# zhiqwang/yolort

Measured on NVIDIA H100. Metric: images/sec end-to-end (letterbox->NMS), higher is better.
Workload: dtype f16

## Files before the change

yolort_b200/csrc/conv_sm90.cu:

```cuda
#include <cstdlib>

#include "common.cuh"
#include "conv_sm90.h"
#include "conv_epilogue.cuh"
#include "conv_chain.cuh"
#include "decode_common.cuh"

namespace yb {

namespace {

constexpr int kMaxStages = 12;
__host__ __device__ constexpr int tile_rows(int groups) { return 64 * groups; }
__host__ __device__ constexpr int cta_threads(int groups) { return 128 * (1 + groups); }
__host__ __device__ constexpr int stage_buf_bytes(int groups) { return tile_rows(groups) * 128; }
constexpr int kStageBufs = 2;
constexpr int kMaxBlockN = 256;
constexpr size_t kSmemBudget = 216 * 1024;
constexpr size_t kStaticSmem = (2 * kMaxStages + 2) * 8 + 2 * kMaxBlockN * 4;
constexpr uint32_t kConsumerBar = 1;

struct ConvKernelParams {
  int M, block_n, block_k;
  int ksize, chunks, num_k_iters;
  int mode;
  int HoWo, Wo, stride, pad;
  int stages;
  int kpg;
  int b_resident;
  uint32_t b_res_bytes;
  int n_tiles, num_tiles;
  int full_tiles, split, num_tasks;
  int ctas;
  int groups;
  int store_cols;
  int bias_len;
  int kk_last;
  uint32_t a_stage_bytes, b_stage_bytes;
  const float* bias;
  EpilogueParams ep;
  ChainParams ch;
  int decode_on;
  int dec_H, dec_W;
  yb_head_decode dec;
};

template <int kGroups>
__device__ __forceinline__ void consumer_sync() { named_bar_sync(kConsumerBar, 128 * kGroups); }

struct ConvTask {
  int m_tile, n_tile, piece, split;
};
template <bool kSplits>
__device__ __forceinline__ ConvTask conv_task(const ConvKernelParams& p, int t) {
  ConvTask k;
  int tile = t;
  k.piece = 0;
  k.split = 1;
  if (kSplits && t >= p.full_tiles) {
    const int u = t - p.full_tiles;
    const int q = u / p.n_tiles;
    tile = p.full_tiles + (q / p.split) * p.n_tiles + (u - q * p.n_tiles);
    k.piece = q % p.split;
    k.split = p.split;
  }
  k.m_tile = tile / p.n_tiles;
  k.n_tile = tile - k.m_tile * p.n_tiles;
  return k;
}

template <bool kBf16, int kW>
__device__ __forceinline__ int stage_mmas(float* acc, const ConvKernelParams& p, uint32_t a_lo0, uint32_t a_step16,
                                          uint32_t b_lo0, uint32_t b_step16, uint64_t ab_hi, int cnt, int ch, int kk,
                                          bool first) {
  for (int j = 0; j < cnt; ++j) {
    const int kc = ch == p.chunks - 1 ? p.kk_last : kk;
    for (int k = 0; k < kc; ++k)
      wgmma_mma<kBf16, kW>(acc, desc_lohi(a_lo0 + j * a_step16 + 2 * k, ab_hi), desc_lohi(b_lo0 + j * b_step16 + 2 * k, ab_hi),
                           !first || (j | k) != 0);
    if (++ch == p.chunks) ch = 0;
  }
  return ch;
}

template <int kN>
__device__ __forceinline__ void decode_fragment(const yb_head_decode& D, const float* acc, const float* s_bias,
                                                const FragRows& fr, int dec_H, int dec_W, float* head, uint32_t wg_bar,
                                                int lane) {
  constexpr int kMaxA = 4;
  const int K = D.n_classes + 5;
  const int q2 = 2 * (lane & 3);
#pragma unroll
  for (int j = 0; j < kN / 8; ++j) {
    {
#pragma unroll
      for (int i = 0; i < 4; ++i) {
        const int col = 8 * j + q2 + (i & 1);
        const int a = col / K, r = col - a * K;
        if (a < D.n_anchors && r < 5) head[fr.loc[i >> 1] * 20 + a * 5 + r] = acc[4 * j + i] + s_bias[col];
      }
    }
  }
  named_bar_sync(wg_bar, 128);
  float obj[2][kMaxA];
  bool pass[2][kMaxA];
  uint32_t emitted[2] = {0u, 0u};
#pragma unroll
  for (int rr = 0; rr < 2; ++rr) {
#pragma unroll
    for (int a = 0; a < kMaxA; ++a) {
      obj[rr][a] = a < D.n_anchors ? sigmoidf_ref(head[fr.loc[rr] * 20 + a * 5 + 4]) : 0.f;
      pass[rr][a] = a < D.n_anchors && fr.ok[rr] && obj[rr][a] > D.score_thresh;
    }
  }
  int n_img[2], py[2], px[2];
  const int hw = dec_H * dec_W;
#pragma unroll
  for (int rr = 0; rr < 2; ++rr) {
    n_img[rr] = static_cast<int>(fr.row[rr] / hw);
    const int rem = static_cast<int>(fr.row[rr] - static_cast<long long>(n_img[rr]) * hw);
    py[rr] = rem / dec_W;
    px[rr] = rem - py[rr] * dec_W;
  }
  const bool any_pass = pass[0][0] || pass[0][1] || pass[0][2] || pass[0][3] || pass[1][0] || pass[1][1] ||
                        pass[1][2] || pass[1][3];
  if (any_pass) {
#pragma unroll
    for (int j = 0; j < kN / 8; ++j) {
      {
#pragma unroll
        for (int i = 0; i < 4; ++i) {
          const int rr = i >> 1;
          const int col = 8 * j + q2 + (i & 1);
          const int a = col / K, r = col - a * K;
          const bool pa = a == 0 ? pass[rr][0] : (a == 1 ? pass[rr][1] : (a == 2 ? pass[rr][2] : (a == 3 && pass[rr][3])));
          if (pa && r >= 5) {
            const float oa = a == 0 ? obj[rr][0] : (a == 1 ? obj[rr][1] : (a == 2 ? obj[rr][2] : obj[rr][3]));
            const float score = __fmul_rn(sigmoidf_ref(acc[4 * j + i] + s_bias[col]), oa);
            if (score > D.score_thresh) {
              const int anchor_flat = D.level_start + (a * dec_H + py[rr]) * dec_W + px[rr];
              emit_candidate(D.keys, D.img_count, D.cap_per_image, n_img[rr], anchor_flat, D.n_classes, r - 5, score);
              emitted[rr] |= 1u << a;
            }
          }
        }
      }
    }
  }
#pragma unroll
  for (int rr = 0; rr < 2; ++rr) {
    emitted[rr] |= __shfl_xor_sync(0xffffffffu, emitted[rr], 1);
    emitted[rr] |= __shfl_xor_sync(0xffffffffu, emitted[rr], 2);
    if ((lane & 3) == 0 && emitted[rr]) {
      const float* h = head + fr.loc[rr] * 20;
      for (int a = 0; a < D.n_anchors; ++a) {
        if (!((emitted[rr] >> a) & 1u)) continue;
        const int anchor_flat = D.level_start + (a * dec_H + py[rr]) * dec_W + px[rr];
        const float4 b = decode_box(sigmoidf_ref(h[a * 5 + 0]), sigmoidf_ref(h[a * 5 + 1]), sigmoidf_ref(h[a * 5 + 2]),
                                    sigmoidf_ref(h[a * 5 + 3]), px[rr], py[rr], D.stride_px, D.anchors_px[2 * a],
                                    D.anchors_px[2 * a + 1]);
        reinterpret_cast<float4*>(D.boxes)[static_cast<long long>(n_img[rr]) * D.anchors_per_image + anchor_flat] = b;
        atomicMax(&D.img_maxc[n_img[rr]], float_to_ordered_int(fmaxf(fmaxf(b.x, b.y), fmaxf(b.z, b.w))));
      }
    }
  }
  named_bar_sync(wg_bar, 128);
}

template <bool kBf16, int kN, bool kDecode, int kN2, int kCtas, int kGroups = 2>
__global__ void __launch_bounds__(cta_threads(kGroups), kCtas)
conv_wgmma_kernel(const __grid_constant__ CUtensorMap tmap_a, const __grid_constant__ CUtensorMap tmap_b,
                  const __grid_constant__ CUtensorMap tmap_out, const __grid_constant__ CUtensorMap tmap_w2,
                  const __grid_constant__ CUtensorMap tmap_out2, const __grid_constant__ CUtensorMap tmap_a64,
                  const __grid_constant__ CUtensorMap tmap_out64, const ConvKernelParams p) {
  static_assert(kGroups == 2 || (kGroups == 1 && kCtas == 2 && !kDecode), "one consumer warpgroup: two CTAs, no decode");
  constexpr bool kChain = kN2 != 0;
  constexpr int kAcc = (kN > kN2 ? kN : kN2) / 2;
  constexpr int kBlockM = tile_rows(kGroups);
  constexpr int kStageBufBytes = stage_buf_bytes(kGroups);
  constexpr bool kSplits = !kDecode && !kChain && kN == 128;
  constexpr bool kRowHalves = kSplits && kGroups == 2;
  extern __shared__ uint8_t smem_raw[];
  __shared__ __align__(8) uint64_t full_bar[kMaxStages];
  __shared__ __align__(8) uint64_t empty_bar[kMaxStages];
  __shared__ __align__(8) uint64_t b_full;
  __shared__ __align__(8) uint64_t w2_full;
  __shared__ __align__(16) float s_bias[kMaxBlockN];
  __shared__ __align__(16) float s_bias2[kChain ? kMaxBlockN : 4];

  uint8_t* tiles = reinterpret_cast<uint8_t*>(
      (reinterpret_cast<uintptr_t>(smem_raw) + 1023) & ~static_cast<uintptr_t>(1023));
  const uint32_t stage_bytes = p.kpg * (p.a_stage_bytes + (p.b_resident ? 0u : p.b_stage_bytes));
  uint8_t* b_res = tiles + static_cast<size_t>(p.stages) * stage_bytes;
  uint8_t* staging = b_res + p.b_res_bytes;
  uint8_t* w2_res = staging + kStageBufs * kStageBufBytes;

  const int warp = threadIdx.x >> 5;
  const int lane = threadIdx.x & 31;

  if (threadIdx.x == 0) {
    tma_prefetch_desc(&tmap_a);
    tma_prefetch_desc(&tmap_b);
    tma_prefetch_desc(&tmap_out);
    for (int s = 0; s < p.stages; ++s) {
      mbar_init(&full_bar[s], 1);
      mbar_init(&empty_bar[s], kGroups);
    }
    mbar_init(&b_full, 1);
    mbar_init(&w2_full, 1);
    mbar_fence_init();
  }
  __syncthreads();

  if (threadIdx.x == 0 && p.b_resident) {
    const uint32_t b_bytes = p.block_n * p.block_k * 2;
    const int n0 = (blockIdx.x % p.n_tiles) * p.block_n;
    mbar_expect_tx(&b_full, p.num_k_iters * b_bytes);
    for (int it = 0; it < p.num_k_iters; ++it)
      tma_load_2d(&tmap_b, &b_full, b_res + it * p.b_stage_bytes, it * p.block_k, n0);
  }
  if constexpr (kChain) {
    if (threadIdx.x == 0) {
      tma_prefetch_desc(&tmap_w2);
      tma_prefetch_desc(&tmap_out2);
      mbar_expect_tx(&w2_full, p.ch.w2_chunks * p.ch.n2 * p.ch.w2_row_bytes);
      for (int j = 0; j < p.ch.w2_chunks; ++j)
        tma_load_2d(&tmap_w2, &w2_full, w2_res + j * p.ch.w2_sub_bytes, j * (p.ch.w2_row_bytes >> 1), 0);
    }
  }
  asm volatile("griddepcontrol.wait;" ::: "memory");
  asm volatile("griddepcontrol.launch_dependents;" ::: "memory");

  if (warp < 4) {
    regs_producer<kCtas, kGroups>();
    if (warp != 0) return;
    const uint32_t a_bytes = kBlockM * p.block_k * 2, b_bytes = p.block_n * p.block_k * 2;
    int kit = 0;
    for (int t = blockIdx.x; t < p.num_tasks; t += gridDim.x) {
      const ConvTask task = conv_task<kSplits>(p, t);
      const bool rows64 = kRowHalves && task.split != 1;
      const int n0 = task.n_tile * p.block_n;
      const int m0 = task.m_tile * kBlockM + (rows64 ? task.piece * 64 : 0);
      const CUtensorMap* map_a = rows64 ? &tmap_a64 : &tmap_a;
      const uint32_t a_task_bytes = rows64 ? a_bytes / 2 : a_bytes;
      int cw = 0, ch = 0, cn = 0;
      if (p.mode == 1) {
        cn = m0 / p.HoWo;
        const int rem = m0 - cn * p.HoWo;
        const int ho = rem / p.Wo;
        const int wo = rem - ho * p.Wo;
        ch = ho * p.stride - p.pad;
        cw = wo * p.stride - p.pad;
      }
      for (int it0 = 0; it0 < p.num_k_iters; it0 += p.kpg, ++kit) {
        const int cnt = min(p.kpg, p.num_k_iters - it0);
        const int s = kit % p.stages;
        const uint32_t ph = (kit / p.stages) & 1;
        mbar_wait(&empty_bar[s], ph ^ 1);
        uint8_t* a_dst = tiles + s * stage_bytes;
        uint8_t* b_dst = a_dst + p.kpg * p.a_stage_bytes;
        if (YB_ELECT()) {
          mbar_expect_tx(&full_bar[s], cnt * (a_task_bytes + (p.b_resident ? 0u : b_bytes)));
          for (int j = 0; j < cnt; ++j) {
            const int it = it0 + j;
            const int tap = it / p.chunks;
            const int chunk = it - tap * p.chunks;
            if (p.mode == 0) {
              tma_load_2d(map_a, &full_bar[s], a_dst + j * p.a_stage_bytes, chunk * p.block_k, m0);
            } else {
              const int r = tap / p.ksize;
              const int sx = tap - r * p.ksize;
              tma_load_im2col_4d(map_a, &full_bar[s], a_dst + j * p.a_stage_bytes, chunk * p.block_k, cw, ch, cn,
                                 static_cast<uint16_t>(sx), static_cast<uint16_t>(r));
            }
            if (!p.b_resident) tma_load_2d(&tmap_b, &full_bar[s], b_dst + j * p.b_stage_bytes, it * p.block_k, n0);
          }
        }
      }
    }
    return;
  }

  regs_consumer<kCtas, kGroups>();
  const int g = (warp >> 2) - 1;
  const int wq = warp & 3;
  const bool issuer = threadIdx.x == 128;
  const int ctid = threadIdx.x - 128;
  FragRows fr;
  fr.loc[0] = g * 64 + wq * 16 + (lane >> 2);
  fr.loc[1] = fr.loc[0] + 8;
  const uint32_t row_bytes = p.block_k * 2;
  const uint32_t ab_hi = desc_hi(row_bytes, 8 * row_bytes);
  const uint32_t a_half16 = (64 * row_bytes) >> 4;
  const uint32_t a_step16 = p.a_stage_bytes >> 4, b_step16 = p.b_stage_bytes >> 4;
  const uint32_t b_res_lo0 = smem_lo16(b_res);
  const int kk = p.block_k >> 4;
  constexpr int bn = kN;
  const int store_cols = p.store_cols;
  float acc[kAcc];

  if constexpr (kChain) {
    for (int i = ctid; i < p.ch.n2; i += 128 * kGroups) s_bias2[i] = (i < p.ch.bias2_len) ? __ldg(p.ch.bias2 + i) : 0.f;
  }
  const bool fixed_n = (gridDim.x % p.n_tiles) == 0;
  if (fixed_n) {
    const int n0f = (blockIdx.x % p.n_tiles) * p.block_n;
    for (int i = ctid; i < p.block_n; i += 128 * kGroups) s_bias[i] = (n0f + i < p.bias_len) ? __ldg(p.bias + n0f + i) : 0.f;
  }
  consumer_sync<kGroups>();
  if (p.b_resident) mbar_wait(&b_full, 0);
  if constexpr (kChain) mbar_wait(&w2_full, 0);

  int kit = 0, store_idx = 0;
  for (int t = blockIdx.x; t < p.num_tasks; t += gridDim.x) {
    const ConvTask task = conv_task<kSplits>(p, t);
    const bool half = kSplits && task.split != 1;
    const bool rows64 = kRowHalves && half;
    const int width = half ? bn / 2 : bn;
    const int col0 = half ? (rows64 ? g : task.piece) * width : 0;
    const int n0 = task.n_tile * p.block_n + col0;
    const int m0 = task.m_tile * kBlockM + (rows64 ? task.piece * 64 : 0);
    const bool load_bias = !fixed_n || (half && !rows64);
    if (load_bias) {
      consumer_sync<kGroups>();
      const int nb = rows64 ? n0 - col0 : n0, wb = rows64 ? bn : width;
      for (int i = ctid; i < wb; i += 128 * kGroups) s_bias[i] = (nb + i < p.bias_len) ? __ldg(p.bias + nb + i) : 0.f;
    }
    const float* bias_cols = s_bias + (rows64 ? col0 : 0);
    const uint32_t b_piece16 = (col0 * row_bytes) >> 4;
    const uint32_t a_group16 = rows64 ? 0u : g * a_half16;

    int chunk = 0, prev_s = -1;
    for (int it0 = 0; it0 < p.num_k_iters; it0 += p.kpg, ++kit) {
      const int cnt = min(p.kpg, p.num_k_iters - it0);
      const int s = kit % p.stages;
      mbar_wait(&full_bar[s], (kit / p.stages) & 1);
      const uint32_t a_lo0 = smem_lo16(tiles + s * stage_bytes) + a_group16;
      const uint32_t b_lo0 =
          (p.b_resident ? b_res_lo0 + it0 * b_step16 : smem_lo16(tiles + s * stage_bytes) + p.kpg * a_step16) + b_piece16;
      wgmma_fence();
      int ch;
      if (!kSplits || width == bn)
        ch = stage_mmas<kBf16, kN>(acc, p, a_lo0, a_step16, b_lo0, b_step16, ab_hi, cnt, chunk, kk, it0 == 0);
      else
        ch = stage_mmas<kBf16, kSplits ? kN / 2 : kN>(acc, p, a_lo0, a_step16, b_lo0, b_step16, ab_hi, cnt, chunk, kk, it0 == 0);
      wgmma_commit();
      wgmma_wait<1>();
      if (prev_s >= 0 && (threadIdx.x & 127) == 0) mbar_arrive(&empty_bar[prev_s]);
      prev_s = s;
      chunk = ch;
    }
    wgmma_wait<0>();
    fence_acc<kN / 2>(acc);
    if ((threadIdx.x & 127) == 0) mbar_arrive(&empty_bar[prev_s]);
    if (load_bias) consumer_sync<kGroups>();

    fr.row[0] = static_cast<long long>(m0) + fr.loc[0] - (rows64 ? g * 64 : 0);
    fr.row[1] = static_cast<long long>(m0) + fr.loc[1] - (rows64 ? g * 64 : 0);
    fr.ok[0] = fr.row[0] < p.M;
    fr.ok[1] = fr.row[1] < p.M;
    if constexpr (kDecode) {
      decode_fragment<kN>(p.dec, acc, s_bias, fr, p.dec_H, p.dec_W, reinterpret_cast<float*>(staging), 2 + g, lane);
    } else {
    if constexpr (kChain) {
      if (issuer) tma_store_wait_read<0>();
      consumer_sync<kGroups>();
    }
    for (int c0 = 0; c0 < width; c0 += store_cols, ++store_idx) {
      uint8_t* buf = staging + (kChain ? (c0 / store_cols) : (store_idx & 1)) * kStageBufBytes;
      epilogue_box<kBf16, kN>(p.ep, acc, c0, store_cols, bias_cols, fr, n0, buf, lane);
      fence_proxy_async_smem();
      if constexpr (!kChain) {
        if (issuer) tma_store_wait_read<0>();
      }
      consumer_sync<kGroups>();
      if (issuer) {
        if (rows64) {
          const int nt = task.n_tile * p.block_n;
          if (m0 < p.M) {
            if (nt + c0 < p.ep.Cout) tma_store_2d(&tmap_out64, buf, nt + c0, m0);
            if (nt + width + c0 < p.ep.Cout) tma_store_2d(&tmap_out64, buf + 64 * store_cols * 2, nt + width + c0, m0);
          }
        } else if ((!kChain || p.ch.store_first) && n0 + c0 < p.ep.Cout) {
          tma_store_2d(&tmap_out, buf, n0 + c0, m0);
        }
        tma_store_commit();
      }
    }
    if constexpr (kChain) {
      const uint32_t a2_hi = desc_hi(p.ch.own_row_bytes, 8 * p.ch.own_row_bytes);
      const uint32_t w2_hi = desc_hi(p.ch.w2_row_bytes, 8 * p.ch.w2_row_bytes);
      const uint32_t stag_lo = smem_lo16(staging) + ((64 * g * p.ch.own_row_bytes) >> 4);
      const uint32_t w2_lo0 = smem_lo16(w2_res);
      wgmma_fence();
      for (int j = 0; j < p.ch.own_chunks; ++j)
        for (int k = 0; k < p.ch.ksteps; ++k)
          wgmma_mma<kBf16, kChain ? kN2 : 16>(acc, desc_lohi(stag_lo + j * (kStageBufBytes >> 4) + 2 * k, a2_hi),
                            desc_lohi(w2_lo0 + j * (p.ch.w2_sub_bytes >> 4) + 2 * k, w2_hi), (j | k) != 0);
      wgmma_commit();
      wgmma_wait<0>();
      fence_acc<kChain ? kN2 / 2 : 8>(acc);
      if (issuer) tma_store_wait_read<0>();
      consumer_sync<kGroups>();
      const int s2 = chain_store2_cols(p.ch.n2);
      for (int c0 = 0; c0 < p.ch.n2; c0 += s2) {
        uint8_t* buf = staging + ((c0 / s2) & 1) * kStageBufBytes;
        epilogue_box<kBf16, kChain ? kN2 : 16>(p.ch.ep2, acc, c0, s2, s_bias2, fr, 0, buf, lane);
        fence_proxy_async_smem();
        if (issuer) tma_store_wait_read<0>();
        consumer_sync<kGroups>();
        if (issuer) {
          if (c0 < p.ch.ep2.Cout) tma_store_2d(&tmap_out2, buf, c0, m0);
          tma_store_commit();
        }
      }
    }
    }
  }
  if (issuer) tma_store_wait_all<0>();
}

using ConvKernelFn = void (*)(const CUtensorMap, const CUtensorMap, const CUtensorMap, const CUtensorMap, const CUtensorMap,
                              const CUtensorMap, const CUtensorMap, const ConvKernelParams);

template <bool kBf16>
ConvKernelFn select_conv_kernel_t(const ConvKernelParams& kp) {
  if (kp.groups == 1) {
    if (kp.ctas != 2 || kp.decode_on || kp.ch.on) return nullptr;
    return kp.block_n == 128 ? conv_wgmma_kernel<kBf16, 128, false, 0, 2, 1> : nullptr;
  }
  if (kp.ctas == 2) {
    if (kp.decode_on) return nullptr;
    if (kp.ch.on) {
      if (kp.block_n != 64) return nullptr;
      return kp.ch.n2 == 32 ? conv_wgmma_kernel<kBf16, 64, false, 32, 2>
                            : (kp.ch.n2 == 64 ? conv_wgmma_kernel<kBf16, 64, false, 64, 2> : nullptr);
    }
    switch (kp.block_n) {
      case 16: return conv_wgmma_kernel<kBf16, 16, false, 0, 2>;
      case 32: return conv_wgmma_kernel<kBf16, 32, false, 0, 2>;
      case 64: return conv_wgmma_kernel<kBf16, 64, false, 0, 2>;
      default: return nullptr;
    }
  }
  if (kp.decode_on) return conv_wgmma_kernel<kBf16, 256, true, 0, 1>;
  if (kp.ch.on) {
    if (kp.block_n == 64)
      return kp.ch.n2 == 32 ? conv_wgmma_kernel<kBf16, 64, false, 32, 1>
                            : (kp.ch.n2 == 64 ? conv_wgmma_kernel<kBf16, 64, false, 64, 1> : conv_wgmma_kernel<kBf16, 64, false, 128, 1>);
    return kp.ch.n2 == 32 ? conv_wgmma_kernel<kBf16, 128, false, 32, 1>
                          : (kp.ch.n2 == 64 ? conv_wgmma_kernel<kBf16, 128, false, 64, 1> : conv_wgmma_kernel<kBf16, 128, false, 128, 1>);
  }
  switch (kp.block_n) {
    case 16: return conv_wgmma_kernel<kBf16, 16, false, 0, 1>;
    case 32: return conv_wgmma_kernel<kBf16, 32, false, 0, 1>;
    case 64: return conv_wgmma_kernel<kBf16, 64, false, 0, 1>;
    case 128: return conv_wgmma_kernel<kBf16, 128, false, 0, 1>;
    default: return conv_wgmma_kernel<kBf16, 256, false, 0, 1>;
  }
}
ConvKernelFn select_conv_kernel(const ConvKernelParams& kp) {
  return kp.ep.is_bf16 ? select_conv_kernel_t<true>(kp) : select_conv_kernel_t<false>(kp);
}

}

static int conv_plan(const yb_op_desc& d, int ctas, int groups, ConvKernelParams& kp, dim3& grid, size_t& smem_bytes);

int conv_validate(const yb_op_desc& d) {
  YB_REQUIRE(d.dtype == YB_F16 || d.dtype == YB_BF16, "conv: dtype must be f16 or bf16");
  YB_REQUIRE((d.reserved & ~(31 | YB_CONV_NO_TAIL_SPLIT | YB_CONV_PAIR_N64 | YB_CONV_NO_TEAMS)) == 0,
             "conv: reserved bits 5 and 9 and up must be zero, got 0x%x",
             d.reserved);
  YB_REQUIRE(d.ksize >= 1 && d.ksize <= 7 && d.stride >= 1 && d.stride <= 2, "conv: ksize/stride");
  YB_REQUIRE(d.act >= YB_ACT_NONE && d.act <= YB_ACT_RELU, "conv: unknown activation %d", d.act);
  YB_REQUIRE(d.Cin % 8 == 0 && d.in_cstride % 8 == 0 && d.in_cstride >= d.Cin,
             "conv: Cin/in_cstride must be multiples of 8 (16-byte TMA granularity), got %d/%d", d.Cin,
             d.in_cstride);
  YB_REQUIRE(d.Cout % 8 == 0 && d.out_cstride % 8 == 0 && d.out_cstride >= d.Cout,
             "conv: Cout/out_cstride must be multiples of 8, got %d/%d", d.Cout, d.out_cstride);
  YB_REQUIRE(d.Cin_pad % 16 == 0 && d.Cin_pad >= d.Cin, "conv: Cin_pad must be a multiple of 16");
  YB_REQUIRE(d.Cout_pad % 16 == 0 && d.Cout_pad >= d.Cout, "conv: Cout_pad must be a multiple of 16");
  YB_REQUIRE((reinterpret_cast<uintptr_t>(d.in) & 15) == 0 && (reinterpret_cast<uintptr_t>(d.out) & 15) == 0 &&
                 (reinterpret_cast<uintptr_t>(d.weight) & 15) == 0,
             "conv: tensors must be 16-byte aligned");
  YB_REQUIRE(d.residual == nullptr ||
                 ((reinterpret_cast<uintptr_t>(d.residual) & 15) == 0 && d.res_cstride % 8 == 0),
             "conv: residual alignment");
  int M;
  return conv_rows(d, "conv", &M);
}

static int conv_configure(const yb_op_desc& d, ConvKernelParams& kp, dim3& grid, size_t& smem_bytes) {
  const int rc = conv_validate(d);
  if (rc != YB_OK) return rc;
  YB_REQUIRE(!(d.reserved & YB_CONV_BAND_STEM),
             "conv: banded stem weights (reserved bit 1) need the halo-patch kernel, which this %dx%d map does not qualify for",
             d.H, d.W);
  if (!(d.reserved & YB_CONV_ONE_CTA) &&
      (conv_plan(d, 2, 2, kp, grid, smem_bytes) == YB_OK || conv_plan(d, 2, 1, kp, grid, smem_bytes) == YB_OK))
    return YB_OK;
  return conv_plan(d, 1, 2, kp, grid, smem_bytes);
}

static int conv_plan(const yb_op_desc& d, int ctas, int groups, ConvKernelParams& kp, dim3& grid, size_t& smem_bytes) {
  const int Ho = d.Ho, Wo = d.Wo;
  const size_t budget = ctas == 2 ? smem_per_sm() / 2 - kSmemReservedPerCta - kStaticSmem : kSmemBudget;
  const int block_m = tile_rows(groups);
  kp = ConvKernelParams();
  kp.ctas = ctas;
  kp.groups = groups;
  kp.M = static_cast<int>(static_cast<long long>(d.N) * Ho * Wo);
  kp.ep.Cout = d.Cout;
  const int m_tiles = (kp.M + block_m - 1) / block_m;
  const int sms = num_sms();
  const int m_tiles128 = (kp.M + tile_rows(2) - 1) / tile_rows(2);
  int block_n = conv_block_n(d.Cout, m_tiles128, d.chain != nullptr);
  if (groups == 1) {
    if (block_n != 256 || d.chain != nullptr || m_tiles128 < 3 * sms) return YB_ERR_INVALID;
    block_n = 128;
  }
  if (groups == 2 && ctas == 1 && block_n == 256 && d.chain == nullptr && d.decode == nullptr &&
      !(d.reserved & (YB_CONV_NO_TAIL_SPLIT | YB_CONV_ONE_CTA)) && static_cast<size_t>(d.ksize) * d.ksize * d.Cin_pad * 256 * 2 > 80 * 1024 &&
      m_tiles > sms && m_tiles < 4 * sms && m_tiles % sms != 0) {
    const int n128 = (d.Cout + 127) / 128, r128 = (m_tiles * n128) % sms;
    if (sms % n128 == 0 && r128 > 0 && 2 * r128 <= sms) block_n = 128;
  }
  int n_tiles = (d.Cout + block_n - 1) / block_n;
  YB_REQUIRE(mma_n(block_n) == block_n && block_n <= kMaxBlockN, "conv: N tile %d is not a wgmma N", block_n);
  kp.block_n = block_n;
  kp.n_tiles = n_tiles;
  kp.num_tiles = m_tiles * n_tiles;
  kp.block_k = (d.Cin_pad % 64 == 0) ? 64 : ((d.Cin_pad % 32 == 0) ? 32 : 16);
  kp.ksize = d.ksize;
  kp.chunks = d.Cin_pad / kp.block_k;
  kp.num_k_iters = d.ksize * d.ksize * kp.chunks;
  kp.mode = (d.ksize == 1 && d.stride == 1 && d.pad == 0) ? 0 : 1;
  kp.HoWo = Ho * Wo;
  kp.Wo = Wo;
  kp.stride = d.stride;
  kp.pad = d.pad;
  kp.decode_on = 0;
  if (d.decode != nullptr) {
    const yb_head_decode& dd = *d.decode;
    const int width = dd.n_anchors * (dd.n_classes + 5);
    if (!(dd.n_anchors > 0 && dd.n_anchors <= 4 && width <= kMaxBlockN && width <= d.Cout_pad && d.ksize == 1 &&
          dd.keys && dd.boxes && dd.img_count && dd.img_maxc)) {
      set_error("conv: fused decode needs a 1x1 head with n_anchors*(n_classes+5) <= %d and a candidate arena", kMaxBlockN);
      return YB_ERR_INVALID;
    }
    n_tiles = 1;
    block_n = mma_n(d.Cout);
    YB_REQUIRE(block_n == 256, "conv: the fused decode is built for heads of 129-256 columns, got %d", d.Cout);
    kp.block_n = block_n;
    kp.n_tiles = 1;
    kp.num_tiles = m_tiles;
    kp.decode_on = 1;
    kp.dec = dd;
    kp.dec_H = Ho;
    kp.dec_W = Wo;
  }
  kp.store_cols = (block_n % 64 == 0) ? 64 : ((block_n % 32 == 0) ? 32 : 16);
  kp.bias_len = d.Cout_pad;
  kp.kk_last = (d.Cin - (kp.chunks - 1) * kp.block_k + 15) / 16;
  if (kp.kk_last < 1) kp.kk_last = 1;
  if (kp.kk_last > (kp.block_k >> 4)) kp.kk_last = kp.block_k >> 4;
  kp.a_stage_bytes = block_m * kp.block_k * 2;
  kp.b_stage_bytes = (static_cast<uint32_t>(kp.block_n * kp.block_k * 2) + 1023u) & ~1023u;
  kp.ch.on = 0;
  size_t chain_bytes = 0;
  if (d.chain != nullptr) {
    YB_REQUIRE(kp.store_cols == 64, "conv: a chained tail needs 64-column output boxes (Cout %% 64 == 0), got Cout=%d", d.Cout);
    const char* why = chain_setup(d, kp.block_n, kp.n_tiles, kp.store_cols, false, &kp.ch);
    YB_REQUIRE(why == nullptr, "conv: chained tail not supported here: %s", why);
    const int s2 = chain_store2_cols(kp.ch.n2);
    YB_REQUIRE(s2 == 64 || s2 == 32, "conv: the tail's Cout_pad must be a multiple of 32, got %d", kp.ch.n2);
    YB_REQUIRE((kp.block_n == 64 || kp.block_n == 128) && kp.ch.n2 <= 128,
               "conv: chained tails are built for N tiles of 64 / 128 and tails of at most 128 columns (block_n=%d, n2=%d)",
               kp.block_n, kp.ch.n2);
    chain_bytes = static_cast<size_t>(kp.ch.w2_chunks) * kp.ch.w2_sub_bytes;
  }
  const size_t fixed = static_cast<size_t>(kStageBufs) * stage_buf_bytes(groups) + 1024 + chain_bytes;
  const bool fixed_n = n_tiles == 1 || (groups == 1 && (2 * sms) % n_tiles == 0);
  KPipeline pipe;
  const int rc = size_k_pipeline(budget, fixed, kp.a_stage_bytes, kp.b_stage_bytes, kp.num_k_iters, fixed_n, kMaxStages,
                                 "conv", kp.block_n, &pipe);
  if (rc != YB_OK) return rc;
  kp.b_resident = pipe.b_resident;
  kp.b_res_bytes = pipe.b_res_bytes;
  kp.kpg = pipe.kpg;
  kp.stages = pipe.stages;
  kp.ep.is_bf16 = d.dtype == YB_BF16;
  kp.ep.act = d.act;
  kp.bias = d.bias;
  kp.ep.residual = d.residual;
  kp.ep.res_cstride = d.res_cstride;
  if (ctas == 2 && (select_conv_kernel(kp) == nullptr || kp.num_tiles < 2 * sms)) return YB_ERR_INVALID;
  if (groups == 1) {
    ConvKernelParams two = kp;
    two.groups = 2;
    if (!kp.b_resident || select_conv_kernel(two) != nullptr) return YB_ERR_INVALID;
  }
  const int max_grid = ctas * sms;
  grid = dim3(kp.num_tiles < max_grid ? kp.num_tiles : max_grid, 1, 1);
  const int G = static_cast<int>(grid.x);
  const int r = kp.num_tiles % G;
  kp.split = !(d.reserved & YB_CONV_NO_TAIL_SPLIT) && !kp.decode_on && !kp.ch.on && kp.block_n == 128 &&
                     G % kp.n_tiles == 0 && r > 0 && 2 * r <= G ? 2 : 1;
  kp.full_tiles = kp.split > 1 ? kp.num_tiles - r : kp.num_tiles;
  kp.num_tasks = kp.full_tiles + (kp.num_tiles - kp.full_tiles) * kp.split;
  smem_bytes = pipe.smem;
  return YB_OK;
}

int im2col_conv_config(const yb_op_desc& d, yb_conv_info* info) {
  ConvKernelParams kp;
  dim3 grid;
  size_t smem = 0;
  const int rc = conv_configure(d, kp, grid, smem);
  if (rc == YB_OK && info) {
    info->kernel = YB_CONV_KERNEL_IM2COL;
    info->block_n = kp.block_n;
    info->n_tiles = kp.n_tiles;
    info->weights_resident = kp.b_resident;
    info->tiles_per_pass = 1;
    info->slots = kp.stages;
    info->ring = kp.kpg;
    info->store_cols = kp.store_cols;
    info->store_bufs = kStageBufs;
    info->groups = kp.groups;
    info->resident_ctas = kp.ctas;
    info->chained = kp.ch.on;
    info->smem_bytes = static_cast<int>(smem);
    info->grid = static_cast<int>(grid.x);
    info->tiling = YB_CONV_TILING_ROWS;
    info->m_tiles = kp.num_tiles / kp.n_tiles;
    info->work_items = kp.num_tiles;
    info->tail_n = kp.ch.n2;
    info->tail_tiles = kp.split > 1 ? kp.num_tiles - kp.full_tiles : 0;
    info->tail_split = kp.split;
  }
  return rc;
}

struct Im2colConvOp final : ConvOp {
  CUtensorMap tmap_a, tmap_b, tmap_out, tmap_w2, tmap_out2, tmap_a64, tmap_out64;
  ConvKernelParams kp;
  ConvKernelFn fn = nullptr;
  dim3 grid;
  size_t smem_bytes;
  int launch(cudaStream_t stream) const override {
    YB_CHECK_CUDA(launch_pdl(fn, grid, dim3(cta_threads(kp.groups)), smem_bytes, stream, tmap_a, tmap_b, tmap_out, tmap_w2,
                             tmap_out2, tmap_a64, tmap_out64, kp));
    return YB_OK;
  }
};

int im2col_conv_create(const yb_op_desc& d, ConvOp** out) {
  Im2colConvOp* op = new Im2colConvOp();
  ConvKernelParams& kp = op->kp;
  int rc = conv_configure(d, kp, op->grid, op->smem_bytes);
  const uint32_t block_m = tile_rows(kp.groups);
  const CUtensorMapDataType dt = kp.ep.is_bf16 ? CU_TENSOR_MAP_DATA_TYPE_BFLOAT16 : CU_TENSOR_MAP_DATA_TYPE_FLOAT16;
  if (rc == YB_OK)
    rc = kp.mode == 0 ? tmap_matrix(&op->tmap_a, "conv input", dt, d.in, d.Cin, kp.M, d.in_cstride, kp.block_k, block_m,
                                    CU_TENSOR_MAP_L2_PROMOTION_L2_128B)
                      : tmap_im2col(&op->tmap_a, "conv input", dt, d, kp.block_k, block_m);
  const int ktot = d.ksize * d.ksize * d.Cin_pad;
  if (rc == YB_OK)
    rc = tmap_matrix(&op->tmap_b, "conv weights", dt, d.weight, ktot, d.Cout_pad, ktot, kp.block_k, kp.block_n,
                     CU_TENSOR_MAP_L2_PROMOTION_L2_256B);
  if (rc == YB_OK)
    rc = tmap_matrix(&op->tmap_out, "conv output", dt, d.out, d.Cout, kp.M, d.out_cstride, kp.store_cols, block_m,
                     CU_TENSOR_MAP_L2_PROMOTION_NONE);
  op->tmap_w2 = op->tmap_b;
  op->tmap_out2 = op->tmap_out;
  op->tmap_a64 = op->tmap_a;
  op->tmap_out64 = op->tmap_out;
  if (rc == YB_OK && kp.split > 1 && kp.groups == 2) {
    rc = kp.mode == 0 ? tmap_matrix(&op->tmap_a64, "conv input (tail halves)", dt, d.in, d.Cin, kp.M, d.in_cstride,
                                    kp.block_k, 64, CU_TENSOR_MAP_L2_PROMOTION_L2_128B)
                      : tmap_im2col(&op->tmap_a64, "conv input (tail halves)", dt, d, kp.block_k, 64);
    if (rc == YB_OK)
      rc = tmap_matrix(&op->tmap_out64, "conv output (tail halves)", dt, d.out, d.Cout, kp.M, d.out_cstride, kp.store_cols,
                       64, CU_TENSOR_MAP_L2_PROMOTION_NONE);
  }
  if (rc == YB_OK && kp.ch.on) {
    const yb_conv_chain& c = *d.chain;
    rc = tmap_matrix(&op->tmap_w2, "conv chained tail weights", dt, c.weight, c.K_pad, c.Cout_pad, c.K_pad,
                     kp.ch.w2_row_bytes / 2, kp.ch.n2, CU_TENSOR_MAP_L2_PROMOTION_L2_256B);
    if (rc == YB_OK)
      rc = tmap_matrix(&op->tmap_out2, "conv chained tail output", dt, c.out, c.Cout, kp.M, c.out_cstride,
                       chain_store2_cols(kp.ch.n2), block_m, CU_TENSOR_MAP_L2_PROMOTION_NONE);
  }
  if (rc == YB_OK) {
    op->fn = select_conv_kernel(kp);
    rc = set_smem_attributes(reinterpret_cast<const void*>(op->fn), kSmemBudget, kp.ctas, op->smem_bytes,
                             cta_threads(kp.groups), "conv");
  }
  if (rc != YB_OK) {
    delete op;
    return rc;
  }
  *out = op;
  return YB_OK;
}

}
```

Before: 8587.

## Add two-team persistent conv kernel overlapping mainloop with chained epilogue

Adds a 640-thread conv kernel for the one-CTA chained 1x1 conv case (N=128 with a 64-column tail). One producer warp feeds two independent A-rings, and two consumer teams of two warpgroups each alternate over 128-row tiles with their own named barriers. While one team runs its epilogue and the chained second GEMM, the other team can run its mainloop. The kernel keeps the B and W2 weights resident and fits fewer pipeline stages per team, adds an occupancy check, and applies only when there are at least 8 tiles per SM.

```diff
diff --git a/yolort_b200/csrc/conv_sm90.cu b/yolort_b200/csrc/conv_sm90.cu
--- a/yolort_b200/csrc/conv_sm90.cu
+++ b/yolort_b200/csrc/conv_sm90.cu
@@ -420,11 +420,208 @@
   if (issuer) tma_store_wait_all<0>();
 }
 
-using ConvKernelFn = void (*)(const CUtensorMap, const CUtensorMap, const CUtensorMap, const CUtensorMap, const CUtensorMap,
+constexpr int kTeamThreads = 640;
+constexpr int kTeamMaxStages = 6;
+constexpr int kTeamMinTilesPerSm = 8;
+constexpr uint32_t kTeamBar0 = 2;
+constexpr size_t kTeamStaticSmem = (4 * kTeamMaxStages + 2) * 8 + 2 * 128 * 4;
+constexpr size_t kTeamSmemBudget = 227 * 1024 - kTeamStaticSmem;
+
+template <bool kBf16, int kN, int kN2>
+__global__ void __launch_bounds__(kTeamThreads, 1)
+conv_wgmma_team_kernel(const __grid_constant__ CUtensorMap tmap_a, const __grid_constant__ CUtensorMap tmap_b,
+                       const __grid_constant__ CUtensorMap tmap_out, const __grid_constant__ CUtensorMap tmap_w2,
+                       const __grid_constant__ CUtensorMap tmap_out2, const __grid_constant__ CUtensorMap tmap_a64,
+                       const __grid_constant__ CUtensorMap tmap_out64, const ConvKernelParams p) {
+  static_assert(kN == 128 && kN2 == 64, "team instances: N = 128 with a 64-column tail");
+  constexpr int kStageBufBytes = stage_buf_bytes(2);
+  extern __shared__ uint8_t smem_raw[];
+  __shared__ __align__(8) uint64_t full_bar[2][kTeamMaxStages];
+  __shared__ __align__(8) uint64_t empty_bar[2][kTeamMaxStages];
+  __shared__ __align__(8) uint64_t b_full;
+  __shared__ __align__(8) uint64_t w2_full;
+  __shared__ __align__(16) float s_bias[kN];
+  __shared__ __align__(16) float s_bias2[kN2];
+
+  uint8_t* tiles = reinterpret_cast<uint8_t*>(
+      (reinterpret_cast<uintptr_t>(smem_raw) + 1023) & ~static_cast<uintptr_t>(1023));
+  const uint32_t ring_bytes = static_cast<uint32_t>(p.stages) * p.a_stage_bytes;
+  uint8_t* b_res = tiles + 2 * ring_bytes;
+  uint8_t* staging = b_res + p.b_res_bytes;
+  uint8_t* w2_res = staging + 2 * kStageBufs * kStageBufBytes;
+
+  const int warp = threadIdx.x >> 5;
+  const int lane = threadIdx.x & 31;
+
+  if (threadIdx.x == 0) {
+    tma_prefetch_desc(&tmap_a);
+    tma_prefetch_desc(&tmap_b);
+    tma_prefetch_desc(&tmap_out);
+    for (int r = 0; r < 2; ++r) {
+      for (int s = 0; s < p.stages; ++s) {
+        mbar_init(&full_bar[r][s], 1);
+        mbar_init(&empty_bar[r][s], 2);
+      }
+    }
+    mbar_init(&b_full, 1);
+    mbar_init(&w2_full, 1);
+    mbar_fence_init();
+  }
+  __syncthreads();
+
+  if (threadIdx.x == 0) {
+    const uint32_t b_bytes = p.block_n * p.block_k * 2;
+    mbar_expect_tx(&b_full, p.num_k_iters * b_bytes);
+    for (int it = 0; it < p.num_k_iters; ++it) tma_load_2d(&tmap_b, &b_full, b_res + it * p.b_stage_bytes, it * p.block_k, 0);
+    tma_prefetch_desc(&tmap_w2);
+    tma_prefetch_desc(&tmap_out2);
+    mbar_expect_tx(&w2_full, p.ch.w2_chunks * p.ch.n2 * p.ch.w2_row_bytes);
+    for (int j = 0; j < p.ch.w2_chunks; ++j)
+      tma_load_2d(&tmap_w2, &w2_full, w2_res + j * p.ch.w2_sub_bytes, j * (p.ch.w2_row_bytes >> 1), 0);
+  }
+  asm volatile("griddepcontrol.wait;" ::: "memory");
+  asm volatile("griddepcontrol.launch_dependents;" ::: "memory");
+  if (warp < 4) {
+    asm volatile("setmaxnreg.dec.sync.aligned.u32 24;\n" ::: "memory");
+    if (warp != 0) return;
+    const uint32_t a_bytes = p.a_stage_bytes;
+    int kit0 = 0, kit1 = 0;
+    for (int t = blockIdx.x, k = 0; t < p.num_tiles; t += gridDim.x, ++k) {
+      const int r = k & 1;
+      const int m0 = t * 128;
+      int kit = r ? kit1 : kit0;
+      for (int it = 0; it < p.num_k_iters; ++it, ++kit) {
+        const int s = kit % p.stages;
+        mbar_wait(&empty_bar[r][s], ((kit / p.stages) & 1) ^ 1);
+        if (YB_ELECT()) {
+          mbar_expect_tx(&full_bar[r][s], a_bytes);
+          tma_load_2d(&tmap_a, &full_bar[r][s], tiles + r * ring_bytes + s * a_bytes, it * p.block_k, m0);
+        }
+      }
+      (r ? kit1 : kit0) = kit;
+    }
+    return;
+  }
+  asm volatile("setmaxnreg.inc.sync.aligned.u32 112;\n" ::: "memory");
+
+  const int cw = (warp >> 2) - 1;
+  const int team = cw >> 1, half = cw & 1;
+  const int wq = warp & 3;
+  const int ctid = threadIdx.x - 128;
+  const bool issuer = (ctid & 255) == 0;
+  const bool wg_leader = (threadIdx.x & 127) == 0;
+  const uint32_t team_bar = kTeamBar0 + team;
+  FragRows fr;
+  fr.loc[0] = half * 64 + wq * 16 + (lane >> 2);
+  fr.loc[1] = fr.loc[0] + 8;
+  uint8_t* team_staging = staging + static_cast<size_t>(team) * kStageBufs * kStageBufBytes;
+  uint8_t* ring = tiles + team * ring_bytes;
+  float acc[kN / 2];
+
+  for (int i = ctid; i < kN; i += 512) s_bias[i] = (i < p.bias_len) ? __ldg(p.bias + i) : 0.f;
+  for (int i = ctid; i < kN2; i += 512) s_bias2[i] = (i < p.ch.bias2_len) ? __ldg(p.ch.bias2 + i) : 0.f;
+  named_bar_sync(kConsumerBar, 512);
+  mbar_wait(&b_full, 0);
+  mbar_wait(&w2_full, 0);
+
+  int kit = 0;
+  for (int t = blockIdx.x + team * gridDim.x; t < p.num_tiles; t += 2 * gridDim.x) {
+    const int m0 = t * 128;
+    {
+      const uint32_t ab_hi = desc_hi(128, 8 * 128);
+      const uint32_t a_wg16 = (64 * 128 * half) >> 4;
+      const uint32_t b_lo0 = smem_lo16(b_res);
+      const uint32_t b_step16 = p.b_stage_bytes >> 4;
+#pragma unroll
+      for (int i = 0; i < kN / 2; ++i) acc[i] = 0.f;
+      int prev_s = -1;
+      for (int it = 0; it < p.num_k_iters; ++it, ++kit) {
+        const int s = kit % p.stages;
+        mbar_wait(&full_bar[team][s], (kit / p.stages) & 1);
+        const uint32_t a_lo = smem_lo16(ring + s * p.a_stage_bytes) + a_wg16;
+        const uint32_t b_lo = b_lo0 + it * b_step16;
+        wgmma_fence();
+#pragma unroll
+        for (int k = 0; k < 4; ++k)
+          wgmma_mma<kBf16, kN>(acc, desc_lohi(a_lo + 2 * k, ab_hi), desc_lohi(b_lo + 2 * k, ab_hi), it != 0 || k != 0);
+        wgmma_commit();
+        wgmma_wait<1>();
+        if (prev_s >= 0 && wg_leader) mbar_arrive(&empty_bar[team][prev_s]);
+        prev_s = s;
+      }
+      wgmma_wait<0>();
+      fence_acc<kN / 2>(acc);
+      if (wg_leader) mbar_arrive(&empty_bar[team][prev_s]);
+    }
+
+#pragma unroll
+    for (int rr = 0; rr < 2; ++rr) {
+      fr.row[rr] = static_cast<long long>(m0) + fr.loc[rr];
+      fr.ok[rr] = fr.row[rr] < p.M;
+    }
+    if (issuer) tma_store_wait_read<0>();
+    named_bar_sync(team_bar, 256);
+#pragma unroll
+    for (int c0 = 0; c0 < kN; c0 += 64) {
+      uint8_t* buf = team_staging + (c0 / 64) * kStageBufBytes;
+      epilogue_box<kBf16, kN>(p.ep, acc, c0, 64, s_bias, fr, 0, buf, lane);
+      fence_proxy_async_smem();
+      named_bar_sync(team_bar, 256);
+      if (issuer) {
+        if (p.ch.store_first && c0 < p.ep.Cout) tma_store_2d(&tmap_out, buf, c0, m0);
+        tma_store_commit();
+      }
+    }
+    {
+      const uint32_t a2_hi = desc_hi(128, 8 * 128);
+      const uint32_t w2_hi = desc_hi(p.ch.w2_row_bytes, 8 * p.ch.w2_row_bytes);
+      const uint32_t stag_lo = smem_lo16(team_staging) + ((64 * half * 128) >> 4);
+      const uint32_t w2_lo0 = smem_lo16(w2_res);
+      const uint32_t w2_step16 = p.ch.w2_sub_bytes >> 4;
+      wgmma_fence();
+      if (p.ch.own_chunks == 2) {
+#pragma unroll
+        for (int j = 0; j < 2; ++j)
+#pragma unroll
+          for (int k = 0; k < 4; ++k)
+            wgmma_mma<kBf16, kN2>(acc, desc_lohi(stag_lo + j * (kStageBufBytes >> 4) + 2 * k, a2_hi),
+                                  desc_lohi(w2_lo0 + j * w2_step16 + 2 * k, w2_hi), (j | k) != 0);
+      } else {
+#pragma unroll
+        for (int k = 0; k < 4; ++k)
+          wgmma_mma<kBf16, kN2>(acc, desc_lohi(stag_lo + 2 * k, a2_hi), desc_lohi(w2_lo0 + 2 * k, w2_hi), k != 0);
+      }
+      wgmma_commit();
+      wgmma_wait<0>();
+      fence_acc<kN2 / 2>(acc);
+    }
+    if (issuer) tma_store_wait_read<0>();
+    named_bar_sync(team_bar, 256);
+    EpilogueParams ep2 = p.ch.ep2;
+    ep2.residual = nullptr;
+#pragma unroll
+    for (int c0 = 0; c0 < kN2; c0 += 64) {
+      uint8_t* buf = team_staging + ((c0 / 64) & 1) * kStageBufBytes;
+      epilogue_box<kBf16, kN2>(ep2, acc, c0, 64, s_bias2, fr, 0, buf, lane);
+      fence_proxy_async_smem();
+      if (issuer) tma_store_wait_read<0>();
+      named_bar_sync(team_bar, 256);
+      if (issuer) {
+        if (c0 < p.ch.ep2.Cout) tma_store_2d(&tmap_out2, buf, c0, m0);
+        tma_store_commit();
+      }
+    }
+  }
+  if (issuer) tma_store_wait_all<0>();
+}
+
+using ConvKernelFn =void (*)(const CUtensorMap, const CUtensorMap, const CUtensorMap, const CUtensorMap, const CUtensorMap,
                               const CUtensorMap, const CUtensorMap, const ConvKernelParams);
 
 template <bool kBf16>
 ConvKernelFn select_conv_kernel_t(const ConvKernelParams& kp) {
+  if (kp.groups == 4)
+    return kp.block_n == 128 && kp.ch.n2 == 64 ? conv_wgmma_team_kernel<kBf16, 128, 64> : nullptr;
   if (kp.groups == 1) {
     if (kp.ctas != 2 || kp.decode_on || kp.ch.on) return nullptr;
     return kp.block_n == 128 ? conv_wgmma_kernel<kBf16, 128, false, 0, 2, 1> : nullptr;
@@ -466,6 +663,7 @@
 }
 
 static int conv_plan(const yb_op_desc& d, int ctas, int groups, ConvKernelParams& kp, dim3& grid, size_t& smem_bytes);
+static void conv_team_plan(ConvKernelParams& kp, size_t& smem_bytes);
 
 int conv_validate(const yb_op_desc& d) {
   YB_REQUIRE(d.dtype == YB_F16 || d.dtype == YB_BF16, "conv: dtype must be f16 or bf16");
@@ -500,7 +698,27 @@
   if (!(d.reserved & YB_CONV_ONE_CTA) &&
       (conv_plan(d, 2, 2, kp, grid, smem_bytes) == YB_OK || conv_plan(d, 2, 1, kp, grid, smem_bytes) == YB_OK))
     return YB_OK;
-  return conv_plan(d, 1, 2, kp, grid, smem_bytes);
+  const int rc1 = conv_plan(d, 1, 2, kp, grid, smem_bytes);
+  if (rc1 == YB_OK && !(d.reserved & (YB_CONV_ONE_CTA | YB_CONV_NO_TEAMS | YB_CONV_PAIR_N64)))
+    conv_team_plan(kp, smem_bytes);
+  return rc1;
+}
+
+static void conv_team_plan(ConvKernelParams& kp, size_t& smem_bytes) {
+  if (!(kp.ctas == 1 && kp.groups == 2 && kp.mode == 0 && kp.ch.on && !kp.decode_on && kp.b_resident &&
+        kp.n_tiles == 1 && kp.block_n == 128 && kp.ch.n2 == 64 && kp.block_k == 64 && kp.kk_last == 4 &&
+        kp.ch.ksteps == 4 && kp.num_tiles >= kTeamMinTilesPerSm * num_sms()))
+    return;
+  const size_t fixed = kp.b_res_bytes + 2 * kStageBufs * static_cast<size_t>(stage_buf_bytes(2)) +
+                       static_cast<size_t>(kp.ch.w2_chunks) * kp.ch.w2_sub_bytes + 1024;
+  if (fixed >= kTeamSmemBudget) return;
+  int stages = static_cast<int>((kTeamSmemBudget - fixed) / (2 * static_cast<size_t>(kp.a_stage_bytes)));
+  if (stages < 2) return;
+  if (stages > kTeamMaxStages) stages = kTeamMaxStages;
+  kp.groups = 4;
+  kp.kpg = 1;
+  kp.stages = stages;
+  smem_bytes = fixed + 2 * static_cast<size_t>(stages) * kp.a_stage_bytes;
 }
 
 static int conv_plan(const yb_op_desc& d, int ctas, int groups, ConvKernelParams& kp, dim3& grid, size_t& smem_bytes) {
@@ -660,7 +878,8 @@
   Im2colConvOp* op = new Im2colConvOp();
   ConvKernelParams& kp = op->kp;
   int rc = conv_configure(d, kp, op->grid, op->smem_bytes);
-  const uint32_t block_m = tile_rows(kp.groups);
+  const bool teams = kp.groups == 4;
+  const uint32_t block_m = tile_rows(teams ? 2 : kp.groups);
   const CUtensorMapDataType dt = kp.ep.is_bf16 ? CU_TENSOR_MAP_DATA_TYPE_BFLOAT16 : CU_TENSOR_MAP_DATA_TYPE_FLOAT16;
   if (rc == YB_OK)
     rc = kp.mode == 0 ? tmap_matrix(&op->tmap_a, "conv input", dt, d.in, d.Cin, kp.M, d.in_cstride, kp.block_k, block_m,
@@ -695,8 +914,21 @@
   }
   if (rc == YB_OK) {
     op->fn = select_conv_kernel(kp);
-    rc = set_smem_attributes(reinterpret_cast<const void*>(op->fn), kSmemBudget, kp.ctas, op->smem_bytes,
-                             cta_threads(kp.groups), "conv");
+    rc = set_smem_attributes(reinterpret_cast<const void*>(op->fn), teams ? kTeamSmemBudget : kSmemBudget, kp.ctas,
+                             op->smem_bytes, cta_threads(kp.groups), "conv");
+    if (rc == YB_OK && teams) {
+      int per_sm = 0;
+      const cudaError_t e =
+          cudaOccupancyMaxActiveBlocksPerMultiprocessor(&per_sm, op->fn, cta_threads(kp.groups), op->smem_bytes);
+      if (e != cudaSuccess) {
+        set_error("conv: cudaOccupancyMaxActiveBlocksPerMultiprocessor failed: %s", cudaGetErrorString(e));
+        rc = YB_ERR_CUDA;
+      } else if (per_sm < 1) {
+        set_error("conv: the two-team CTA (%d threads, %zu bytes of shared memory) does not fit on an SM",
+                  cta_threads(kp.groups), op->smem_bytes);
+        rc = YB_ERR_INVALID;
+      }
+    }
   }
   if (rc != YB_OK) {
     delete op;
```

New measurement: 8974 (median of 6 runs). 1.05x the previous value.
